# ofrikleinfeld/ObjectPermanence

Measured on AMD Instinct MI355X. Metric: CATER clips/sec (300f x 10obj) OPNet inference, higher is better.
Workload: dtype f32

## Files before the change

include/opnet_hip.h:

```cpp
#ifndef OPNET_HIP_H
#define OPNET_HIP_H

#include <stddef.h>
#include <stdint.h>

#ifdef __cplusplus
extern "C" {
#endif

#define OPNET_OK 0
#define OPNET_EINVAL (-1)
#define OPNET_ESHAPE (-2)
#define OPNET_EWORKSPACE (-3)
#define OPNET_EHIP (-4)

#define OPNET_SLOTS 15
#define OPNET_FEATS 6

#define OPNET_HIP_ABI_VERSION 9
int opnet_hip_abi_version(void);
const char *opnet_last_error(void);

size_t opnet_packed_weights_bytes(int H1, int H2);
int opnet_pack_weights_f32(const float *w_ih1, const float *w_hh1, const float *w_sel,
                           const float *w_ih2, const float *w_hh2, const float *w_out,
                           float *packed, size_t packed_bytes, int H1, int H2, void *stream);

size_t opnet_workspace_bytes(int B, int T, int H1, int H2);
int opnet_forward_f32(const float *boxes, const float *packed, float *y, float *logits,
                      void *workspace, size_t workspace_bytes, int B, int T, int H1, int H2,
                      void *stream);

typedef struct opnet_plan opnet_plan;
int opnet_plan_create(opnet_plan **plan, int B, int T, int H1, int H2);
int opnet_plan_forward(opnet_plan *plan, const float *boxes, const float *packed, float *y,
                       float *logits, void *workspace, size_t workspace_bytes, void *stream);
void opnet_plan_destroy(opnet_plan *plan);

int opnet_xcd_max_batch(void);
int opnet_xcd_supported(int H1, int H2);
size_t opnet_xcd_workspace_bytes(int B, int T, int H1, int H2);
int opnet_xcd_forward_f32(const float *boxes, const float *packed, float *y, float *logits,
                          void *workspace, size_t workspace_bytes, int B, int T, int H1, int H2,
                          void *stream);
int opnet_xcd_forward_multi_f32(const float *const *boxes, const int *counts, int nreq, const float *packed, float *y,
                                float *logits, void *workspace, size_t workspace_bytes, int T, int H1, int H2, void *stream);
int opnet_xcd_profile(int enable);
int opnet_xcd_profile_read(double *kernel_ms_total, int *launches);
int opnet_kernel_profile_read(int tag, double *kernel_ms_total, int *launches);
void opnet_xcd_set_trace(void *device_buffer);
int opnet_xcd4_max_batch(void);
size_t opnet_xcd4_packed_weights_bytes(int H1, int H2);
size_t opnet_xcd4_workspace_bytes(int B, int T, int H1, int H2);
int opnet_xcd4_pack_weights_f32(const float *w_ih1, const float *w_hh1, const float *w_sel, const float *w_ih2,
                                const float *w_hh2, const float *w_out, float *packed, size_t packed_bytes,
                                int H1, int H2, void *stream);
int opnet_xcd4_forward_f32(const float *boxes, const float *packed, float *y, float *logits, void *workspace,
                           size_t workspace_bytes, int B, int T, int H1, int H2, void *stream);
void opnet_xcd4_set_trace(void *device_buffer);
int opnet_xcd4_last_status(unsigned *out4);
size_t opnet_xcd4_status_offset(int B, int T, int H1, int H2);
size_t opnet_train_status_offset(int B, int T, int H1, int H2);
void opnet_xcd4_enable(int on);
int opnet_xcd4_enabled(void);

size_t opnet_train_packed_weights_bytes(int H1, int H2);
int opnet_train_pack_weights_f32(const float *w_ih1, const float *w_hh1, const float *w_sel,
                                 const float *w_ih2, const float *w_hh2, const float *w_out,
                                 float *packed, size_t packed_bytes, int H1, int H2, void *stream);
size_t opnet_train_workspace_bytes(int B, int T, int H1, int H2);
int opnet_train_forward_f32(const float *boxes, const float *packed, float *y, float *logits,
                            void *workspace, size_t workspace_bytes, int B, int T, int H1, int H2,
// ... 259 lines not shown
```

objectpermanence_amd/_lib.py:

```python
from __future__ import annotations

import ctypes
import os
from ctypes import POINTER, c_char_p, c_double, c_float, c_int, c_size_t, c_void_p

from . import build as _build

_LIB = None

OPNET_OK = 0
ABI_VERSION = 9
NO_OFFSET = ctypes.c_size_t(-1).value


class OpnetHipError(RuntimeError):
    pass


def _declare(lib):
    fp = c_void_p
    lib.opnet_hip_abi_version.restype = c_int
    lib.opnet_hip_abi_version.argtypes = []
    lib.opnet_last_error.restype = c_char_p
    lib.opnet_last_error.argtypes = []
    lib.opnet_packed_weights_bytes.restype = c_size_t
    lib.opnet_packed_weights_bytes.argtypes = [c_int, c_int]
    lib.opnet_pack_weights_f32.restype = c_int
    lib.opnet_pack_weights_f32.argtypes = [fp, fp, fp, fp, fp, fp, fp, c_size_t, c_int, c_int, c_void_p]
    lib.opnet_workspace_bytes.restype = c_size_t
    lib.opnet_workspace_bytes.argtypes = [c_int, c_int, c_int, c_int]
    lib.opnet_forward_f32.restype = c_int
    lib.opnet_forward_f32.argtypes = [fp, fp, fp, fp, c_void_p, c_size_t, c_int, c_int, c_int, c_int, c_void_p]
    lib.opnet_xcd_max_batch.restype = c_int
    lib.opnet_xcd_max_batch.argtypes = []
    lib.opnet_xcd_supported.restype = c_int
    lib.opnet_xcd_supported.argtypes = [c_int, c_int]
    lib.opnet_xcd_workspace_bytes.restype = c_size_t
    lib.opnet_xcd_workspace_bytes.argtypes = [c_int, c_int, c_int, c_int]
    lib.opnet_xcd_forward_f32.restype = c_int
    lib.opnet_xcd_forward_f32.argtypes = [fp, fp, fp, fp, c_void_p, c_size_t, c_int, c_int, c_int, c_int, c_void_p]
    lib.opnet_xcd_forward_multi_f32.restype = c_int
    lib.opnet_xcd_forward_multi_f32.argtypes = [POINTER(c_void_p), POINTER(c_int), c_int, fp, fp, fp, c_void_p, c_size_t,
                                                c_int, c_int, c_int, c_void_p]
    lib.opnet_xcd_profile.restype = c_int
    lib.opnet_xcd_profile.argtypes = [c_int]
    lib.opnet_xcd_profile_read.restype = c_int
    lib.opnet_xcd_profile_read.argtypes = [POINTER(c_double), POINTER(c_int)]
    lib.opnet_kernel_profile_read.restype = c_int
    lib.opnet_kernel_profile_read.argtypes = [c_int, POINTER(c_double), POINTER(c_int)]
    lib.opnet_xcd_set_trace.restype = None
    lib.opnet_xcd_set_trace.argtypes = [c_void_p]
    lib.opnet_xcd4_max_batch.restype = c_int
    lib.opnet_xcd4_max_batch.argtypes = []
    lib.opnet_xcd4_packed_weights_bytes.restype = c_size_t
    lib.opnet_xcd4_packed_weights_bytes.argtypes = [c_int, c_int]
    lib.opnet_xcd4_workspace_bytes.restype = c_size_t
    lib.opnet_xcd4_workspace_bytes.argtypes = [c_int, c_int, c_int, c_int]
    lib.opnet_xcd4_pack_weights_f32.restype = c_int
    lib.opnet_xcd4_pack_weights_f32.argtypes = [fp, fp, fp, fp, fp, fp, fp, c_size_t, c_int, c_int, c_void_p]
    lib.opnet_xcd4_forward_f32.restype = c_int
    lib.opnet_xcd4_forward_f32.argtypes = [fp, fp, fp, fp, c_void_p, c_size_t, c_int, c_int, c_int, c_int, c_void_p]
    lib.opnet_xcd4_set_trace.restype = None
    lib.opnet_xcd4_set_trace.argtypes = [c_void_p]
    lib.opnet_xcd4_last_status.restype = c_int
    lib.opnet_xcd4_last_status.argtypes = [POINTER(ctypes.c_uint)]
    lib.opnet_plan_create.restype = c_int
    lib.opnet_plan_create.argtypes = [POINTER(c_void_p), c_int, c_int, c_int, c_int]
# ... 254 lines not shown
    lib.opdet_detections_workspace_bytes.restype = c_size_t
    lib.opdet_detections_workspace_bytes.argtypes = [c_int, c_int]
    lib.opdet_detections_f32.restype = c_int
    lib.opdet_detections_f32.argtypes = [fp, fp, fp, fp, c_int, c_int, c_int, c_int, c_int, c_int, c_float, c_float, c_int,
                                         fp, fp, fp, fp, c_void_p, c_size_t, c_void_p]
    lib.opdet_rpn_workspace_bytes_batch.restype = c_size_t
    lib.opdet_rpn_workspace_bytes_batch.argtypes = [c_int, c_int, ip, ip, ip, c_int, c_int, c_int]
    lib.opdet_rpn_proposals_batch_f32.restype = c_int
    lib.opdet_rpn_proposals_batch_f32.argtypes = [POINTER(c_void_p), c_int, c_int, ip, ip, ip, c_int, c_int, c_int, c_int, c_int, c_int,
                                                  c_float, c_float, fp, fp, fp, c_void_p, c_size_t, c_void_p]
    lib.opdet_roi_align_batch_f32.restype = c_int
    lib.opdet_roi_align_batch_f32.argtypes = [POINTER(c_void_p), c_int, ip, ip, c_int, c_int, fp, fp, c_int, fp, c_void_p]
    lib.opdet_detections_workspace_bytes_batch.restype = c_size_t
    lib.opdet_detections_workspace_bytes_batch.argtypes = [c_int, c_int, c_int]
    lib.opdet_detections_batch_f32.restype = c_int
    lib.opdet_detections_batch_f32.argtypes = [fp, fp, fp, fp] + [c_int] * 9 + [c_float, c_float, c_int,
                                               fp, fp, fp, fp, c_void_p, c_size_t, c_void_p]
    lib.opnet_encode_clips_f32.restype = c_int
    lib.opnet_encode_clips_f32.argtypes = [c_void_p, c_void_p, c_void_p, c_void_p, c_void_p, c_int, c_int, c_int, c_void_p, c_int,
                                           c_void_p, c_void_p]
    lib.opnet_load_clips_f32.restype = c_int
    lib.opnet_load_clips_f32.argtypes = [c_void_p, c_void_p, c_int, c_int, c_int, c_void_p, c_int, c_void_p, c_void_p, c_void_p,
                                         c_char_p, c_int]
    lib.opnet_postprocess_iou.restype = c_int
    lib.opnet_postprocess_iou.argtypes = [fp, fp, fp, fp, fp, c_int, c_int, c_void_p]
    lib.opnet_dp_guard_f32.restype = c_int
    lib.opnet_dp_guard_f32.argtypes = [fp, fp, fp, c_float, c_void_p]


EXPORTS = [
    "opnet_hip_abi_version", "opnet_last_error", "opnet_packed_weights_bytes", "opnet_pack_weights_f32",
    "opnet_workspace_bytes", "opnet_forward_f32", "opnet_plan_create", "opnet_plan_forward",
    "opnet_plan_destroy", "opnet_postprocess_iou", "opnet_encode_clips_f32", "opnet_load_clips_f32",
    "opnet_xcd_max_batch", "opnet_xcd_supported", "opnet_xcd_workspace_bytes", "opnet_xcd_forward_f32", "opnet_xcd_forward_multi_f32", "opnet_xcd_set_trace", "opnet_xcd4_set_trace", "opnet_xcd4_last_status", "opnet_xcd4_max_batch", "opnet_xcd4_packed_weights_bytes",
    "opnet_xcd4_workspace_bytes", "opnet_xcd4_pack_weights_f32", "opnet_xcd4_forward_f32",
    "opnet_xcd_profile", "opnet_xcd_profile_read", "opnet_kernel_profile_read",
    "opnet_train_packed_weights_bytes", "opnet_train_pack_weights_f32", "opnet_train_workspace_bytes",
    "opnet_train_forward_f32", "opnet_train_backward_f32", "opnet_train_extra_workspace_bytes", "opnet_train_backward_ex_f32",
    "opnet_selection_ce_f32", "opnet_l1_loss_f32", "opnet_smooth_l1_loss_f32", "opnet_adam_step_f32", "opnet_adam_multi_step_f32",
    "opnet_adam_multi_step_guarded_f32", "opnet_dp_guard_f32", "opnet_xcd4_status_offset", "opnet_train_status_offset", "opnet_xcd4_enable", "opnet_xcd4_enabled",
    "opnet_mlp_pack_weights_f32", "opnet_mlp_forward_f32",
    "opnet_stream_state_floats", "opnet_stream_workspace_bytes", "opnet_stream_step_f32", "opnet_stream_step_ragged_f32",
    "opnet_stream_x4_max_streams", "opnet_stream_x4_workspace_bytes", "opnet_stream_x4_status_offset",
    "opnet_stream_step_x4_f32",
    "opnet_online_encode_f32", "opnet_online_encode_ragged_f32",
    "opnet_mlp_train_pack_weights_f32", "opnet_mlp_train_forward_f32", "opnet_mlp_train_backward_f32",
    "opnet_mlp_train_backward_ex_f32", "opnet_train_forward_state_f32", "opnet_train_backward_state_f32",
    "opseq_lstm_stack_packed_bytes", "opseq_lstm_stack_workspace_bytes", "opseq_lstm_stack_pack_weights_f32",
    "opseq_lstm_stack_forward_f32", "opseq_lstm_stack_forward_graph_f32", "opseq_graph_cache_clear",
    "opseq_stream_state_floats", "opseq_stream_workspace_bytes", "opseq_stream_step_f32", "opseq_stream_step_ragged_f32",
    "opseq_stream_input_product_f32",
    "opseq_stream_x_max_streams", "opseq_stream_x_workspace_bytes", "opseq_stream_x_status_offset", "opseq_stream_step_x_f32",
    "opseq_xcd_supported", "opseq_xcd_enable", "opseq_xcd_max_batch", "opseq_xcd_packed_bytes", "opseq_xcd_workspace_bytes",
    "opseq_xcd_status_offset", "opseq_xcd_pack_weights_f32", "opseq_xcd_forward_f32", "opseq_lstm_stack_train_status_offset", "opseq_xcd_set_trace",
    "opseq_xcdt_supported", "opseq_xcdt_enable", "opseq_xcdt_max_batch", "opseq_xcdt_packed_bytes", "opseq_xcdt_workspace_bytes",
    "opseq_xcdt_status_offset", "opseq_xcdt_pack_weights_f32", "opseq_xcdt_forward_f32", "opseq_xcdt_set_trace",
    "opseq_slot_embed_relu_f32", "opseq_slot_embed_relu_bwd_f32", "opseq_slot_embed_bwd_workspace_bytes", "opseq_slot_embed_relu_bwd_ws_f32",
    "opseq_lstm_stack_train_packed_bytes", "opseq_lstm_stack_train_workspace_bytes",
    "opseq_lstm_stack_train_pack_weights_f32", "opseq_lstm_stack_train_forward_f32",
    "opseq_lstm_stack_train_backward_f32",
    "opseq_encoder_workspace_bytes",
    "opseq_encoder_layer_f32", "opseq_encoder_layer_segmented_f32", "opseq_encoder_layer_batched_f32", "opseq_ffn_fused_supported", "opseq_ffn_fused_plan", "opseq_ffn_fused_f32", "opseq_attention_f32", "opseq_attention_workspace_bytes",
    "opseq_encoder_train_saved_bytes", "opseq_encoder_train_scratch_bytes", "opseq_encoder_layer_train_forward_f32",
    "opseq_encoder_layer_train_backward_f32", "opseq_encoder_test_masks_set", "opseq_encoder_test_masks_clear",
    "opdet_conv2d_f32", "opdet_conv2d_workspace_bytes", "opdet_conv2d_ws_f32", "opdet_wino_weights_bytes", "opdet_wino_weights_f32", "opdet_conv2d_wino_workspace_bytes", "opdet_conv2d_wino_f32", "opdet_conv2d_up_f32", "opdet_conv2d_dual_workspace_bytes", "opdet_conv2d_dual_f32", "opdet_maxpool3x3s2_f32", "opdet_subsample2_f32", "opdet_upsample_add_f32",
    "opdet_preprocess_frame_f32", "opdet_rpn_workspace_bytes", "opdet_rpn_proposals_f32", "opdet_roi_align_f32",
    "opdet_detections_workspace_bytes", "opdet_detections_f32", "opdet_rpn_workspace_bytes_batch", "opdet_rpn_proposals_batch_f32",
# ... 33 lines not shown
```

objectpermanence_amd/csrc/opnet_abi.hip:

```cpp
#include "opnet_kernels.hip"
#include "opnet_xcd_kernels.hip"
#include "opnet_xcd_split_kernels.hip"
#include "opnet_train_kernels.hip"
#include "opnet_state_train_kernels.hip"
#include "opnet_xcd4_kernels.hip"
#include "seq_kernels.hip"
#include "seq_xcd_kernels.hip"
#include "seq_xcdt_kernels.hip"
#include "seq_xcd_bwd_kernels.hip"
#include "conv_kernels.hip"
#include "wino_kernels.hip"
#include "ffn_kernels.hip"
#include "attn_kernels.hip"
#include "enc_train_kernels.hip"
#include "attn_train_kernels.hip"
#include "opnet_stream_kernels.hip"
#include "opnet_stream_x4_kernels.hip"
#include "seq_stream_kernels.hip"
#include "seq_stream_x_kernels.hip"
#include "online_encode_kernels.hip"

#include <stdarg.h>
#include <stdlib.h>
#include <stdio.h>
// ... 292 lines not shown
static int xcd_ring_mode() { return env_int("OPNET_XCD_RING", 1) != 0; }
static int xcd_head_once(int NGT) { return env_int("OPNET_XCD_HO", (NGT + XCD_COUNT - 1) / XCD_COUNT >= 3 ? 1 : 0) != 0; }
static int xcd_split_mode() { return env_int("OPNET_XCD_SPLIT", 1) != 0; }
static int xcd_pgather_mode() { return env_int("OPNET_XCD_PGATHER", 1) != 0; }
static int xcd_head_once_split() { return env_int("OPNET_XCD_HO", 1) != 0; }

static XcdWorkspaceLayout xcd_workspace_layout(int B, int T, bool infer = false)
{
    XcdWorkspaceLayout L;
    const size_t NGT = (size_t)(B + 15) / 16;
    size_t o = 0;
    L.NGT = (int)NGT;
    L.ring = xcd_ring_mode();
    L.ho = infer && xcd_split_mode() ? xcd_head_once_split() : xcd_head_once(L.NGT);
    const size_t NS = L.ring ? (size_t)XCD_RING : (size_t)(T + 1);
    L.status = o; o += 2048;
    L.flags = o;  o += align_up(NGT * XCD_CUS * 4, 256);
    L.xp = o;     o += NGT * (size_t)(T + 2) * OPNET_KXQ * 256;
    L.h1h = o;    o += NGT * NS * (XCD_H1 / 4) * 256;
    L.h2h = o;    o += NGT * NS * (XCD_H2 / 4) * 256;
    L.fbh = o;    o += NGT * NS * 1024;
    L.yp = o;     if (L.ring && !L.ho) o += NGT * (size_t)T * XCD_CUS * 256;
    L.wsp = L.xs = L.fbs = 0;
    if (infer && L.ho) {
        o = align_up(o, 256);
        L.wsp = o; o += align_up(packed_layout(XCD_H1, XCD_H2).total * 4, 256);
        L.xs = o;  o += NGT * (size_t)(T + 2) * OPNET_KXQ * 256;
        L.fbs = o; o += NGT * NS * 2048;
    }
    L.total = align_up(o, 256);
    return L;
}

#define XCD_MAX_B (XCD_COUNT * XCD_NGMAX * 16)

static int check_xcd(int B, int T, int H1, int H2)
{
    if (B <= 0 || T <= 0) return fail(OPNET_ESHAPE, "B=%d T=%d must be positive", B, T);
    if (H1 != XCD_H1 || H2 != XCD_H2)
        return fail(OPNET_ESHAPE, "the per-XCD persistent forward is built for H1=%d, H2=%d (got %d, %d); use opnet_forward_f32",
                    XCD_H1, XCD_H2, H1, H2);
    if (B > XCD_MAX_B) return fail(OPNET_ESHAPE, "B=%d > %d clips per launch: split the batch", B, XCD_MAX_B);
    const XcdWorkspaceLayout L = xcd_workspace_layout(B, T, true);
    if (L.total >= ((size_t)1 << 31))
        return fail(OPNET_ESHAPE, "B=%d x T=%d: the workspace exceeds the 2 GiB one buffer descriptor addresses; split the batch", B, T);
    return OPNET_OK;
}

extern "C" int opnet_xcd_max_batch(void) { return XCD_MAX_B; }

extern "C" size_t opnet_xcd_workspace_bytes(int B, int T, int H1, int H2)
{
    if (check_xcd(B, T, H1, H2)) return 0;
    return xcd_workspace_layout(B, T, true).total;
}

static unsigned long long *g_xcd_trace = nullptr;
extern "C" void opnet_xcd_set_trace(void *device_buffer) { g_xcd_trace = (unsigned long long *)device_buffer; }

static std::mutex g_xcd_mu;
static hipEvent_t g_xcd_done[64] = {};
#define BWD_MAX_SLICES 4
struct BwdSide {
    hipStream_t s[BWD_MAX_SLICES - 1];
    hipEvent_t fork, join[BWD_MAX_SLICES - 1];
};
static BwdSide g_bwd_side[64] = {};
static int g_xcd_cus[64] = {};

#define PROF_XCD 0
#define PROF_SEQX 1
#define PROF_ATTN 2
#define PROF_SEQT 3
#define PROF_FFN 4
#define PROF_ATTN_TF 5
// ... 62 lines not shown
    std::lock_guard<std::mutex> lock(g_xcd_mu);
    if (!g_xcd_cus[dev]) {
        hipDeviceProp_t prop;
        if (hipGetDeviceProperties(&prop, dev) != hipSuccess) return 0;
        g_xcd_cus[dev] = prop.multiProcessorCount;
    }
    return g_xcd_cus[dev];
}

static bool whole_device(int dev) { return xcd_device_cus(dev) >= XCD_COUNT * XCD_CUS; }
static bool whole_device()
{
    int dev = 0;
    return hipGetDevice(&dev) == hipSuccess && whole_device(dev);
}

static int persistent_device(int *dev)
{
    HIP_TRY(hipGetDevice(dev));
    if (!whole_device(*dev))
        return fail(OPNET_ESHAPE, "device %d exposes %d CUs; a persistent launch needs %d resident workgroups", *dev,
                    xcd_device_cus(*dev), XCD_COUNT * XCD_CUS);
    return OPNET_OK;
}

template <class Launch>
static int persistent_launch(int dev, hipStream_t st, int tag, Launch launch)
{
    if (dev < 0 || dev >= 64) return fail(OPNET_EINVAL, "device index %d out of range", dev);
    std::lock_guard<std::mutex> lock(g_xcd_mu);
    if (!g_xcd_done[dev]) HIP_TRY(hipEventCreateWithFlags(&g_xcd_done[dev], hipEventDisableTiming));
    else HIP_TRY(hipStreamWaitEvent(st, g_xcd_done[dev], 0));
    ProfPair pe{};
    const bool prof = tag >= 0 && prof_begin(st, &pe);
    launch();
    if (prof) prof_end(tag, st, pe);
    HIP_TRY(hipEventRecord(g_xcd_done[dev], st));
    return OPNET_OK;
}

extern "C" int opnet_xcd_supported(int H1, int H2)
{
    if (H1 != XCD_H1 || H2 != XCD_H2) return 0;
    return whole_device() ? 1 : 0;
}

static XcdArgs make_xcd_args(const XcdWorkspaceLayout &L, size_t base, size_t status, int B, int T, const float *packed, char *w,
                             float *y, float *logits)
{
    XcdArgs a;
    memset(&a, 0, sizeof(a));
    a.B = B; a.T = T; a.NGT = L.NGT;
    a.packed = packed;
    a.xp = (const float4 *)(w + base + L.xp);
    a.h1h = (float4 *)(w + base + L.h1h);
    a.h2h = (float4 *)(w + base + L.h2h);
    a.fbh = (float4 *)(w + base + L.fbh);
    a.flags = (unsigned *)(w + base + L.flags);
    a.status = (unsigned *)(w + status);
    a.logits = logits;
    a.ws = w;
    a.xp_off = (unsigned)(base + L.xp); a.h1_off = (unsigned)(base + L.h1h); a.h2_off = (unsigned)(base + L.h2h);
    a.fb_off = (unsigned)(base + L.fbh); a.flags_off = (unsigned)(base + L.flags); a.status_off = (unsigned)status;
    a.ring = L.ring; a.yp_off = (unsigned)(base + L.yp); a.y = y;
    a.force_safe = env_int("OPNET_XCD_SAFE", 0);
    a.debug = env_int("OPNET_XCD_DEBUG", 0);
    return a;
}

template <bool TRAIN>
static int xcd_forward_launch(const XcdSources &src, const XcdArgs &a, bool ho, int dev, hipStream_t st)
{
    opnet_xcd_pack_input<<<dim3(a.T + 2, a.NGT), 384, 0, st>>>(src, a);
    if (int rc = persistent_launch(dev, st, PROF_XCD, [&] {
            if (ho) opnet_xcd_forward<true, TRAIN><<<XCD_COUNT * XCD_CUS, 512, 0, st>>>(a);
            else opnet_xcd_forward<false, TRAIN><<<XCD_COUNT * XCD_CUS, 512, 0, st>>>(a);
        }))
        return rc;
    if (a.ring && ho)
        opnet_xcd_y_poison<<<64, 256, 0, st>>>(a, a.y);
    else if (a.ring)
        opnet_xcd_y_reduce<<<ew_blocks((long)a.NGT * a.T * 16, 2048), 256, 0, st>>>(a, a.y);
    else
        opnet_xcd_out_head<<<dim3(a.T, a.NGT), 256, 0, st>>>(a, a.y);
    HIP_TRY(hipGetLastError());
    return OPNET_OK;
}

static int xcd_forward_launch_split(const XcdSources &src, const XcdArgs &a0, const XcdWorkspaceLayout &L, int dev, hipStream_t st)
{
    XcdSplitArgs s;
    memset(&s, 0, sizeof(s));
    s.a = a0;
    s.a.fbh = (float4 *)(a0.ws + L.fbs);
    s.a.fb_off = (unsigned)L.fbs;
    s.wsp = a0.ws + L.wsp;
    s.xs_off = (unsigned)L.xs;
    s.pgather = xcd_pgather_mode();
    const PackedLayout P = packed_layout(XCD_H1, XCD_H2);
    const long lanes = (long)((P.wih2p + (P.total - P.wselp)) / 512) * 64;
    s.wsp_blocks = (unsigned)((lanes + 255) / 256);
    opnet_xcd_split_weights<<<s.wsp_blocks, 256, 0, st>>>(s);
    opnet_xcd_pack_input_split<<<dim3(s.a.T + 2, s.a.NGT), 384, 0, st>>>(src, s);
    if (int rc = persistent_launch(dev, st, PROF_XCD, [&] { opnet_xcd_forward_split<<<XCD_COUNT * XCD_CUS, 512, 0, st>>>(s); }))
        return rc;
    if (s.a.ring) opnet_xcd_y_poison<<<64, 256, 0, st>>>(s.a, s.a.y);
    else opnet_xcd_out_head_split<<<dim3(s.a.T, s.a.NGT), 256, 0, st>>>(s.a, s.a.y);
    HIP_TRY(hipGetLastError());
    return OPNET_OK;
}

static int xcd_forward_impl(const XcdSources &src, const float *packed, float *y, float *logits,
                            void *workspace, size_t workspace_bytes, int B, int T, int H1, int H2,
                            void *stream)
{
    if (int rc = check_xcd(B, T, H1, H2)) return rc;
    if (!packed || !y || !logits || !workspace) return fail(OPNET_EINVAL, "null pointer");
    if (!aligned16(packed) || !aligned16(y) || !aligned16(workspace))
        return fail(OPNET_EINVAL, "packed/y/workspace must be 16-byte aligned");
    const XcdWorkspaceLayout L = xcd_workspace_layout(B, T, true);
    if (workspace_bytes < L.total) return fail(OPNET_EWORKSPACE, "workspace %zu B < %zu B", workspace_bytes, L.total);
    int dev = 0;
    if (int rc = persistent_device(&dev)) return rc;
    XcdArgs a = make_xcd_args(L, 0, L.status, B, T, packed, (char *)workspace, y, logits);
    a.trace = g_xcd_trace;
    if (L.ho && xcd_split_mode()) return xcd_forward_launch_split(src, a, L, dev, (hipStream_t)stream);
    return xcd_forward_launch<false>(src, a, L.ho, dev, (hipStream_t)stream);
}

extern "C" int opnet_xcd_forward_f32(const float *boxes, const float *packed, float *y, float *logits,
                                     void *workspace, size_t workspace_bytes, int B, int T, int H1, int H2,
                                     void *stream)
{
    if (!boxes) return fail(OPNET_EINVAL, "null pointer");
    if (((uintptr_t)boxes) & 7u) return fail(OPNET_EINVAL, "boxes must be 8-byte aligned");
    XcdSources src;
    memset(&src, 0, sizeof(src));
// ... 175 lines not shown
}

struct TrainPackedLayout {
    size_t fwd_total, w2bt, w1bt, wih2t, wsel, wout, x4fwd, x4bwd, total;
};

static bool x4_dims(int H1, int H2) { return H1 == XCD_H1 && H2 == XCD_H2; }

static TrainPackedLayout train_packed_layout(int H1, int H2)
{
    TrainPackedLayout L;
    size_t o = packed_layout(H1, H2).total;
    L.fwd_total = o;
    o = align_up(o, 4);
    L.w2bt = o;  o += (size_t)(H2 / 16) * (H2 / 4) * 256;
    L.w1bt = o;  o += (size_t)(H1 / 16) * (H1 / 4) * 256;
    L.wih2t = o; o += (size_t)(H2 / 4) * 256;
    L.wsel = o;  o += align_up((size_t)OPNET_SLOTS * H1, 4);
    L.wout = o;  o += align_up((size_t)4 * H2, 4);
    L.x4fwd = o; o += x4_dims(H1, H2) ? x4_packed_layout().total : 0;
    L.x4bwd = o; o += x4_dims(H1, H2) ? x4b_packed_layout().total : 0;
    L.total = o;
    return L;
}

struct TrainWorkspaceLayout {
    size_t io, xp, state, h1all, c1all, h2all, c2all, state_end, x2all, g1, g2, psave, ystage, lgstage,
        dyp, dlall, dhpart2, dhpart1, dx2part, dcz, dc2, dc1, dcz_end, l1part, x4h1x, x4h2x, x4status, x4da1x, x4da2x, x4dfx, wgpart,
        xcdws, total;
};
#define WG2_MAX_WAVES 1024

static bool x4_batch(int B, int H1, int H2) { return x4_dims(H1, H2) && (B + 31) / 32 <= X4_NGMAX; }
static bool xcdt_batch(int B, int H1, int H2) { return x4_dims(H1, H2) && B > 96 && B <= XCD_MAX_B; }

static TrainWorkspaceLayout train_workspace_layout(int B, int T, int H1, int H2)
{
    const size_t RB = (B + 31) / 32, TT = T;
    TrainWorkspaceLayout L;
    size_t o = 0;
    L.io = o;      o += align_up(sizeof(OpnetIO), 256);
    L.xp = o;      o += TT * RB * OPNET_KXQ * 32 * 16;
    L.state = o;
    L.h1all = o;   o += (TT + 1) * RB * (size_t)H1 * 32 * 4;
    L.c1all = o;   o += (TT + 1) * RB * (size_t)H1 * 32 * 4;
    L.h2all = o;   o += (TT + 1) * RB * (size_t)H2 * 32 * 4;
    L.c2all = o;   o += (TT + 1) * RB * (size_t)H2 * 32 * 4;
    L.state_end = o;
    L.x2all = o;   o += TT * RB * 64 * 16;
    L.g1 = o;      o += TT * RB * (size_t)H1 * 32 * 16;
    L.g2 = o;      o += TT * RB * (size_t)H2 * 32 * 16;
    L.psave = o;   o += TT * RB * 128 * 16;
    L.ystage = o;  o += RB * 32 * TT * 16;
    L.lgstage = o; o += RB * 32 * TT * OPNET_SLOTS * 4;
    L.dyp = o;     o += TT * RB * 32 * 16;
    L.dlall = o;   o += TT * RB * 128 * 16;
    L.dhpart2 = o; o += 4 * RB * (size_t)H2 * 32 * 4;
    L.dhpart1 = o; o += 4 * RB * (size_t)H1 * 32 * 4;
    L.dx2part = o; o += 4 * RB * 16 * 32 * 4;
    L.dcz = o;
    L.dc2 = o;     o += RB * (size_t)H2 * 32 * 4;
    L.dc1 = o;     o += RB * (size_t)H1 * 32 * 4;
    L.dcz_end = o;
    L.l1part = o;  o += 1024 * 4;
    o = align_up(o, 4096);
    const size_t NG = x4_batch(B, H1, H2) ? RB * 8 : 0;
    L.x4h1x = o;   o += NG * X4_SLOTS * 4096;
// ... 2388 lines not shown
```

objectpermanence_amd/csrc/opnet_xcd_kernels.hip:

```cpp
#include <hip/hip_runtime.h>
#include <stdint.h>

#include <type_traits>

#include "opnet_ctx.h"

#define XCD_COUNT 8
#define XCD_CUS 32
#define XCD_NGMAX 8
#define XCD_H1 256
#define XCD_H2 512
#define XCD_RING 4
#define XCD_SPIN_LIMIT 150000000ll

#define XB_X0 0
#define XB_H1 (6 * 64)
#define XB_H2 (22 * 64)
#define XB_FB (54 * 64)
#define XB_F4 (55 * 64)
#define XB_CHUNKS 55

struct XcdArgs {
    int B, T, NGT;
    const float *packed;
// ... 30 lines not shown
    unsigned keep;
    asm volatile("s_mov_b32 %0, m0\n\ts_mov_b32 m0, %4\n\ts_nop 2\n\tbuffer_load_dwordx4 %1, %2, %3 offen sc1 lds\n\ts_mov_b32 m0, %0"
                 : "=&s"(keep) : "v"(voff), "s"(rsrc), "s"(soff), "s"(lds_dst) : "memory");
}

__device__ __forceinline__ void xcd_store16(__amdgpu_buffer_rsrc_t r, unsigned voff, unsigned soff, float4 v, bool local)
{
    xcd_u32x4 u;
    u.x = __float_as_uint(v.x); u.y = __float_as_uint(v.y); u.z = __float_as_uint(v.z); u.w = __float_as_uint(v.w);
    if (local) __builtin_amdgcn_raw_buffer_store_b128(u, r, voff, soff, 0);
    else __builtin_amdgcn_raw_buffer_store_b128(u, r, voff, soff, 16);
}
__device__ __forceinline__ void xcd_st4(__amdgpu_buffer_rsrc_t r, unsigned voff, unsigned soff, float4 v)
{
    xcd_u32x4 u;
    u.x = __float_as_uint(v.x); u.y = __float_as_uint(v.y); u.z = __float_as_uint(v.z); u.w = __float_as_uint(v.w);
    __builtin_amdgcn_raw_buffer_store_b128(u, r, voff, soff, 0);
}
__device__ __forceinline__ void xcd_st1(__amdgpu_buffer_rsrc_t r, unsigned voff, unsigned soff, float v)
{
    __builtin_amdgcn_raw_buffer_store_b32(__float_as_uint(v), r, voff, soff, 0);
}
__device__ __forceinline__ void xcd_store4(__amdgpu_buffer_rsrc_t r, unsigned voff, unsigned soff, float v, bool local)
{
    if (local) __builtin_amdgcn_raw_buffer_store_b32(__float_as_uint(v), r, voff, soff, 0);
    else __builtin_amdgcn_raw_buffer_store_b32(__float_as_uint(v), r, voff, soff, 16);
}
__device__ __forceinline__ void xcd_store_flag(unsigned *p, unsigned v, bool local)
{
    if (local) __hip_atomic_store(p, v, __ATOMIC_RELAXED, __HIP_MEMORY_SCOPE_WAVEFRONT);
    else __hip_atomic_store(p, v, __ATOMIC_RELAXED, __HIP_MEMORY_SCOPE_AGENT);
}

#define XCD_MAX_SOURCES 64
struct XcdSources {
    const float *p[XCD_MAX_SOURCES];
    int start[XCD_MAX_SOURCES + 1];
    int n;
};

__global__ void __launch_bounds__(384) opnet_xcd_pack_input(const XcdSources src, XcdArgs a)
{
    const int slot = blockIdx.x, gg = blockIdx.y;
    const int T = a.T, tid = threadIdx.x;
    const float4 z = make_float4(0.f, 0.f, 0.f, 0.f);
    {
        const int kq = tid % OPNET_KXQ, clip = tid / OPNET_KXQ;
        const int b = gg * 16 + clip, t = slot - 1;
        float4 v = z;
        if (b < a.B && t >= 0 && t < T) {
            int r = 0;
            while (r + 1 < src.n && b >= src.start[r + 1]) ++r;
            const float2 *s2 = (const float2 *)(src.p[r] + ((long)(b - src.start[r]) * T + t) * OPNET_KX + kq * 4);
            const int k = kq * 4;
            if (k + 1 < OPNET_KX) { float2 p = s2[0]; v.x = p.x; v.y = p.y; }
            if (k + 3 < OPNET_KX) { float2 q = s2[1]; v.z = q.x; v.w = q.y; }
        }
        ((float4 *)a.xp)[(((long)gg * (T + 2) + slot) * OPNET_KXQ + kq) * 16 + clip] = v;
    }
    if (slot == 0) {
        const long NS = a.ring ? XCD_RING : T + 1;
        float4 *h1 = a.h1h + (long)gg * NS * (XCD_H1 * 4);
        float4 *h2 = a.h2h + (long)gg * NS * (XCD_H2 * 4);
        for (int i = tid; i < XCD_H1 * 4; i += 384) h1[i] = z;
        for (int i = tid; i < XCD_H2 * 4; i += 384) h2[i] = z;
        if (tid < 64) a.fbh[(long)gg * NS * 64 + tid] = z;
        if (tid < XCD_CUS) a.flags[gg * XCD_CUS + tid] = 0u;
        if (gg == 0 && tid < 8) a.status[tid] = 0u;
        if (gg == 0 && tid < XCD_COUNT * XCD_CUS) a.status[8 + tid] = 0xffffffffu;
    }
}

__device__ __forceinline__ bool xcd_flags_ready(const unsigned *flags, unsigned need)
{
    const unsigned v = __hip_atomic_load(flags + (threadIdx.x & 31), __ATOMIC_RELAXED, __HIP_MEMORY_SCOPE_AGENT);
    return __all(v >= need);
}

__device__ __forceinline__ bool xcd_wait_flags(const unsigned *flags, unsigned need, unsigned *status, int phase)
{
    if (xcd_flags_ready(flags, need)) return true;
    const int lane = threadIdx.x & 63;
    long long t0 = 0;
    for (unsigned spins = 1;; ++spins) {
        __builtin_amdgcn_s_sleep(4);
// ... 643 lines not shown
    }
}


__global__ void __launch_bounds__(256) opnet_xcd_y_reduce(const XcdArgs a, float *__restrict__ y)
{
    const long total = (long)a.NGT * a.T * 16;
    const float4 *yp = (const float4 *)(a.ws + a.yp_off);
    const bool bad = a.status[0] != 0u;
    for (long i = blockIdx.x * 256L + threadIdx.x; i < total; i += (long)gridDim.x * 256) {
        const int n = (int)(i & 15);
        const long gt = i >> 4;
        const float4 *p = yp + gt * (XCD_CUS * 16) + n;
        float4 sum = p[0];
        for (int cu = 1; cu < XCD_CUS; ++cu) {
            const float4 v = p[cu * 16];
            sum.x += v.x; sum.y += v.y; sum.z += v.z; sum.w += v.w;
        }
        if (bad) sum = make_float4(NAN, NAN, NAN, NAN);
        const long gg = gt / a.T, t = gt - gg * a.T;
        const long b = gg * 16 + n;
        if (b < a.B) ((float4 *)y)[b * a.T + t] = sum;
    }
}


__global__ void __launch_bounds__(256) opnet_xcd_y_poison(const XcdArgs a, float *__restrict__ y)
{
    if (a.status[0] == 0u) return;
    const long total = (long)a.B * a.T;
    for (long i = blockIdx.x * 256L + threadIdx.x; i < total; i += (long)gridDim.x * 256)
        ((float4 *)y)[i] = make_float4(NAN, NAN, NAN, NAN);
}
```

objectpermanence_amd/csrc/opnet_xcd_split_kernels.hip:

```cpp
#define XS_SCALE 2048.f
#define XS_ISCALE (1.f / 2048.f)
#define XS_RANGE 32768.f
#define XS_ABORT_RANGE 3u
#define XS_CHUNKS 56
#define XS_F8 (XS_CHUNKS * 64)
#define XS_H1 (6 * 64)
#define XS_H2 (22 * 64)

typedef _Float16 xs_h8 __attribute__((ext_vector_type(8)));
typedef _Float16 xs_h4 __attribute__((ext_vector_type(4)));
typedef unsigned xs_u32x2 __attribute__((ext_vector_type(2)));

struct XcdSplitArgs {
    XcdArgs a;
    const char *wsp;
    unsigned xs_off;
    unsigned wsp_blocks;
    int pgather;
};

__device__ __forceinline__ void xs_split(float v, _Float16 *hi, _Float16 *lo)
{
    const _Float16 h = (_Float16)v;
    *hi = h;
// ... 15 lines not shown
        const float4 v0 = src[0], v1 = src[16];
        const float v[8] = {v0.x, v0.y, v0.z, v0.w, v1.x, v1.y, v1.z, v1.w};
        xs_h8 hi, lo;
#pragma unroll
        for (int j = 0; j < 8; ++j) {
            _Float16 h, q;
            xs_split(v[j], &h, &q);
            hi[j] = h; lo[j] = q;
            bad |= !xs_in_range(v[j]);
        }
        xs_h8 *dst = (xs_h8 *)(s.wsp + base * 4) + l;
        dst[0] = hi;
        dst[64] = lo;
    }
    if (i < (long)(P.wselp - P.wih2p)) bad |= !xs_in_range(s.a.packed[P.wih2p + i]);
    const int any = __syncthreads_or(bad ? 1 : 0);
    if (threadIdx.x == 0) ((unsigned *)(s.wsp + P.wih2p * 4))[blockIdx.x] = any ? 1u : 0u;
    if (blockIdx.x == 0) {
        if (threadIdx.x < 8) s.a.status[threadIdx.x] = 0u;
        s.a.status[8 + threadIdx.x] = 0xffffffffu;
    }
}

__global__ void __launch_bounds__(384) opnet_xcd_pack_input_split(const XcdSources src, const XcdSplitArgs s)
{
    const XcdArgs &a = s.a;
    const int slot = blockIdx.x, gg = blockIdx.y;
    const int T = a.T, tid = threadIdx.x;
    const float4 z = make_float4(0.f, 0.f, 0.f, 0.f);
    bool bad = false;
    {
        const int kq = tid % OPNET_KXQ, clip = tid / OPNET_KXQ;
        const int b = gg * 16 + clip, t = slot - 1;
        float4 v = z;
        if (b < a.B && t >= 0 && t < T) {
            int r = 0;
            while (r + 1 < src.n && b >= src.start[r + 1]) ++r;
            const float2 *s2 = (const float2 *)(src.p[r] + ((long)(b - src.start[r]) * T + t) * OPNET_KX + kq * 4);
            const int k = kq * 4;
            if (k + 1 < OPNET_KX) { float2 p = s2[0]; v.x = p.x; v.y = p.y; }
            if (k + 3 < OPNET_KX) { float2 q = s2[1]; v.z = q.x; v.w = q.y; }
        }
        const long sl = (long)gg * (T + 2) + slot;
        ((float4 *)a.xp)[(sl * OPNET_KXQ + kq) * 16 + clip] = v;
        xs_h4 hi, lo;
        const float vv[4] = {v.x, v.y, v.z, v.w};
#pragma unroll
        for (int j = 0; j < 4; ++j) {
            _Float16 h, q;
            xs_split(vv[j], &h, &q);
            hi[j] = h; lo[j] = q;
            bad |= !xs_in_range(vv[j]);
        }
        char *d = a.ws + s.xs_off + sl * (OPNET_KXQ * 256) + (kq >> 3) * 2048 + ((((kq >> 1) & 3) * 16 + clip) * 16) + (kq & 1) * 8;
        *(xs_h4 *)d = hi;
        *(xs_h4 *)(d + 1024) = lo;
    }
    const long NS = a.ring ? XCD_RING : T + 1;
    for (long fs = slot; fs < NS; fs += T + 2)
        if (tid < 128) ((float4 *)(a.ws + a.fb_off))[((long)gg * NS + fs) * 128 + tid] = z;
    if (slot == 0) {
        float4 *h1 = a.h1h + (long)gg * NS * (XCD_H1 * 4);
        float4 *h2 = a.h2h + (long)gg * NS * (XCD_H2 * 4);
        for (int i = tid; i < XCD_H1 * 4; i += 384) h1[i] = z;
        for (int i = tid; i < XCD_H2 * 4; i += 384) h2[i] = z;
        if (tid < XCD_CUS) a.flags[gg * XCD_CUS + tid] = 0u;
        if (gg == 0) {
            const PackedLayout P = packed_layout(XCD_H1, XCD_H2);
            const unsigned *wb = (const unsigned *)(s.wsp + P.wih2p * 4);
            for (unsigned i = tid; i < s.wsp_blocks; i += 384) bad |= wb[i] != 0u;
// ... 477 lines not shown
```

objectpermanence_amd/learned_models.py:

```python
from __future__ import annotations

import math
import os
from typing import Dict, Tuple

import torch
import torch.nn as nn

from . import _lib
from ._device_cache import PackedImages, TrainingBuffers, Workspaces, check_weights
from .launch_monitor import LaunchMonitor


class AbstractCaterModel(nn.Module):

    def __init__(self, config: Dict[str, int]):
        super().__init__()
        self.config: Dict[str, int] = config
        self.max_objects_in_frame = 15
        self.bb_in_dim = 5
        self.bb_out_dim = 4

    def launch_guard(self):
        r = getattr(self, "_runner", None)
# ... 444 lines not shown
    def _forward_xcd4(self, boxes: torch.Tensor, stream: int):
        lib = _lib.load()
        B, T, dev = int(boxes.shape[0]), int(boxes.shape[1]), boxes.device
        x4packed = self._x4_packed_weights(dev, stream)
        ws = self._x4ws.get(stream, (B, T), dev, (lib.opnet_xcd4_workspace_bytes, B, T, self._h1, self._h2))
        y = torch.empty((B, T, 4), dtype=torch.float32, device=dev)
        logits = torch.empty((B, 15, T), dtype=torch.float32, device=dev)
        _lib.check(lib.opnet_xcd4_forward_f32(boxes.data_ptr(), x4packed.data_ptr(), y.data_ptr(), logits.data_ptr(),
                                              ws.data_ptr(), ws.numel(), B, T, self._h1, self._h2, stream),
                   "opnet_xcd4_forward_f32")
        self._monitor.watch(ws, lib.opnet_xcd4_status_offset(B, T, self._h1, self._h2),
                            lambda: self._redo_on_chain(boxes, y, logits), "opnet_xcd4_forward")
        return y, logits

    def _forward_xcd(self, boxes: torch.Tensor, packed: torch.Tensor, stream: int):
        lib = _lib.load()
        B, T, dev = int(boxes.shape[0]), int(boxes.shape[1]), boxes.device
        y = torch.empty((B, T, 4), dtype=torch.float32, device=dev)
        logits = torch.empty((B, 15, T), dtype=torch.float32, device=dev)
        step = int(lib.opnet_xcd_max_batch())
        while step > 64 and lib.opnet_xcd_workspace_bytes(min(step, B), T, self._h1, self._h2) == 0:
            step //= 2
        for lo in range(0, B, step):
            n = min(step, B - lo)
            ws = self._xws.get(stream, (n, T), dev, (lib.opnet_xcd_workspace_bytes, n, T, self._h1, self._h2))
            rc = lib.opnet_xcd_forward_f32(boxes[lo:lo + n].data_ptr(), packed.data_ptr(), y[lo:lo + n].data_ptr(),
                                           logits[lo:lo + n].data_ptr(), ws.data_ptr(), ws.numel(), n, T,
                                           self._h1, self._h2, stream)
            _lib.check(rc, "opnet_xcd_forward_f32")
            self._monitor.watch(ws, 0, lambda b=boxes[lo:lo + n], yy=y[lo:lo + n], ll=logits[lo:lo + n]:
                                self._redo_on_chain(b, yy, ll), "opnet_xcd_forward")
        return y, logits

    def forward_requests(self, requests):
        lib = _lib.load()
        B = sum(int(r.shape[0]) for r in requests)
        ok = (len(requests) > 1 and len(requests) <= 64 and not torch.is_grad_enabled() and all(r.is_cuda for r in requests)
              and not self._wants_xcd4(B) and self._wants_xcd(B) and B <= int(lib.opnet_xcd_max_batch())
              and all(r.dim() == 4 and r.shape[1:] == requests[0].shape[1:] and r.device == requests[0].device for r in requests))
        if not ok:
            return self(requests[0] if len(requests) == 1 else torch.cat(list(requests), dim=0))
        reqs = [r if (r.is_contiguous() and r.dtype == torch.float32) else r.contiguous().float() for r in requests]
        T, dev = int(reqs[0].shape[1]), reqs[0].device
        if reqs[0].shape[2] != 15 or reqs[0].shape[3] != 6:
            raise ValueError(f"boxes must be [B, T, 15, 6], got {tuple(reqs[0].shape)}")
        with torch.cuda.device(dev):
            packed = self._packed_weights(dev)
            stream = _stream_ptr(dev)
            if lib.opnet_xcd_workspace_bytes(B, T, self._h1, self._h2) == 0:
                return self(torch.cat(reqs, dim=0))
            ws = self._xws.get(stream, (B, T), dev, (lib.opnet_xcd_workspace_bytes, B, T, self._h1, self._h2))
            y = torch.empty((B, T, 4), dtype=torch.float32, device=dev)
            logits = torch.empty((B, 15, T), dtype=torch.float32, device=dev)
            n = len(reqs)
            ptrs = (_lib.c_void_p * n)(*[r.data_ptr() for r in reqs])
            counts = (_lib.ctypes.c_int * n)(*[int(r.shape[0]) for r in reqs])
            _lib.check(lib.opnet_xcd_forward_multi_f32(ptrs, counts, n, packed.data_ptr(), y.data_ptr(), logits.data_ptr(),
                                                       ws.data_ptr(), ws.numel(), T, self._h1, self._h2, stream),
                       "opnet_xcd_forward_multi_f32")
            self._monitor.watch(ws, 0, lambda: self._redo_on_chain(torch.cat(reqs, dim=0), y, logits), "opnet_xcd_forward")
        return y, logits

    def xcd_status(self):
        return {k: ws[:12].view(torch.int32).tolist() for k, ws in self._xws.items()}

    def zero_state(self, B: int):
        return _zero_state(self, B)

    def forward(self, boxes: torch.Tensor, logits_grad: bool = False, state=None, return_state: bool = False):
        if not boxes.is_cuda:
# ... 616 lines not shown
```

Measured before the change: 254,800.

## Run oversized XCD batches as multiple persistent-kernel rounds inside one call

```diff
diff --git a/include/opnet_hip.h b/include/opnet_hip.h
--- a/include/opnet_hip.h
+++ b/include/opnet_hip.h
@@ -38,6 +38,7 @@
 void opnet_plan_destroy(opnet_plan *plan);
 
 int opnet_xcd_max_batch(void);
+int opnet_xcd_round_plan(int B, int *first_group, int *groups, int capacity);
 int opnet_xcd_supported(int H1, int H2);
 size_t opnet_xcd_workspace_bytes(int B, int T, int H1, int H2);
 int opnet_xcd_forward_f32(const float *boxes, const float *packed, float *y, float *logits,
diff --git a/objectpermanence_amd/_lib.py b/objectpermanence_amd/_lib.py
--- a/objectpermanence_amd/_lib.py
+++ b/objectpermanence_amd/_lib.py
@@ -33,6 +33,8 @@
     lib.opnet_forward_f32.argtypes = [fp, fp, fp, fp, c_void_p, c_size_t, c_int, c_int, c_int, c_int, c_void_p]
     lib.opnet_xcd_max_batch.restype = c_int
     lib.opnet_xcd_max_batch.argtypes = []
+    lib.opnet_xcd_round_plan.restype = c_int
+    lib.opnet_xcd_round_plan.argtypes = [c_int, POINTER(c_int), POINTER(c_int), c_int]
     lib.opnet_xcd_supported.restype = c_int
     lib.opnet_xcd_supported.argtypes = [c_int, c_int]
     lib.opnet_xcd_workspace_bytes.restype = c_size_t
@@ -353,7 +355,7 @@
     "opnet_hip_abi_version", "opnet_last_error", "opnet_packed_weights_bytes", "opnet_pack_weights_f32",
     "opnet_workspace_bytes", "opnet_forward_f32", "opnet_plan_create", "opnet_plan_forward",
     "opnet_plan_destroy", "opnet_postprocess_iou", "opnet_encode_clips_f32", "opnet_load_clips_f32",
-    "opnet_xcd_max_batch", "opnet_xcd_supported", "opnet_xcd_workspace_bytes", "opnet_xcd_forward_f32", "opnet_xcd_forward_multi_f32", "opnet_xcd_set_trace", "opnet_xcd4_set_trace", "opnet_xcd4_last_status", "opnet_xcd4_max_batch", "opnet_xcd4_packed_weights_bytes",
+    "opnet_xcd_max_batch", "opnet_xcd_round_plan", "opnet_xcd_supported", "opnet_xcd_workspace_bytes", "opnet_xcd_forward_f32", "opnet_xcd_forward_multi_f32", "opnet_xcd_set_trace", "opnet_xcd4_set_trace", "opnet_xcd4_last_status", "opnet_xcd4_max_batch", "opnet_xcd4_packed_weights_bytes",
     "opnet_xcd4_workspace_bytes", "opnet_xcd4_pack_weights_f32", "opnet_xcd4_forward_f32",
     "opnet_xcd_profile", "opnet_xcd_profile_read", "opnet_kernel_profile_read",
     "opnet_train_packed_weights_bytes", "opnet_train_pack_weights_f32", "opnet_train_workspace_bytes",
diff --git a/objectpermanence_amd/csrc/opnet_abi.hip b/objectpermanence_amd/csrc/opnet_abi.hip
--- a/objectpermanence_amd/csrc/opnet_abi.hip
+++ b/objectpermanence_amd/csrc/opnet_abi.hip
@@ -348,7 +348,31 @@
     return L;
 }
 
-#define XCD_MAX_B (XCD_COUNT * XCD_NGMAX * 16)
+#define XCD_LAUNCH_GROUPS (XCD_COUNT * XCD_NGMAX)
+#define XCD_LAUNCH_B (XCD_LAUNCH_GROUPS * 16)
+#define XCD_MAX_ROUNDS 4
+#define XCD_MAX_B (XCD_MAX_ROUNDS * XCD_LAUNCH_B)
+
+static int xcd_round_plan(int NGT, int *first, int *groups)
+{
+    const int R = (NGT + XCD_LAUNCH_GROUPS - 1) / XCD_LAUNCH_GROUPS;
+    const int base = R ? NGT / R : 0, rem = R ? NGT % R : 0;
+    for (int r = 0, g = 0; r < R; ++r) {
+        first[r] = g;
+        groups[r] = base + (r < rem ? 1 : 0);
+        g += groups[r];
+    }
+    return R;
+}
+
+extern "C" int opnet_xcd_round_plan(int B, int *first_group, int *groups, int capacity)
+{
+    if (B <= 0 || B > XCD_MAX_B || !first_group || !groups) return 0;
+    int f[XCD_MAX_ROUNDS], n[XCD_MAX_ROUNDS];
+    const int R = xcd_round_plan((B + 15) / 16, f, n);
+    for (int r = 0; r < R && r < capacity; ++r) { first_group[r] = f[r]; groups[r] = n[r]; }
+    return R;
+}
 
 static int check_xcd(int B, int T, int H1, int H2)
 {
@@ -356,7 +380,7 @@
     if (H1 != XCD_H1 || H2 != XCD_H2)
         return fail(OPNET_ESHAPE, "the per-XCD persistent forward is built for H1=%d, H2=%d (got %d, %d); use opnet_forward_f32",
                     XCD_H1, XCD_H2, H1, H2);
-    if (B > XCD_MAX_B) return fail(OPNET_ESHAPE, "B=%d > %d clips per launch: split the batch", B, XCD_MAX_B);
+    if (B > XCD_MAX_B) return fail(OPNET_ESHAPE, "B=%d > %d clips per call: split the batch", B, XCD_MAX_B);
     const XcdWorkspaceLayout L = xcd_workspace_layout(B, T, true);
     if (L.total >= ((size_t)1 << 31))
         return fail(OPNET_ESHAPE, "B=%d x T=%d: the workspace exceeds the 2 GiB one buffer descriptor addresses; split the batch", B, T);
@@ -485,9 +509,11 @@
     if (!g_xcd_done[dev]) HIP_TRY(hipEventCreateWithFlags(&g_xcd_done[dev], hipEventDisableTiming));
     else HIP_TRY(hipStreamWaitEvent(st, g_xcd_done[dev], 0));
     ProfPair pe{};
-    const bool prof = tag >= 0 && prof_begin(st, &pe);
-    launch();
-    if (prof) prof_end(tag, st, pe);
+    bool prof = tag >= 0 && prof_begin(st, &pe);
+    auto prof_close = [&] { if (prof) { prof_end(tag, st, pe); prof = false; } };
+    if constexpr (std::is_invocable_v<Launch, decltype(prof_close) &>) launch(prof_close);
+    else launch();
+    prof_close();
     HIP_TRY(hipEventRecord(g_xcd_done[dev], st));
     return OPNET_OK;
 }
@@ -521,13 +547,49 @@
     return a;
 }
 
+static XcdArgs xcd_round_view(const XcdArgs &a, int g0, int n, size_t fb_slot)
+{
+    XcdArgs v = a;
+    const size_t G = (size_t)g0, T = (size_t)a.T, NS = a.ring ? (size_t)XCD_RING : T + 1;
+    const size_t xp = G * (T + 2) * OPNET_KXQ * 256, h1 = G * NS * (XCD_H1 / 4) * 256, h2 = G * NS * (XCD_H2 / 4) * 256;
+    const size_t fb = G * NS * fb_slot, fl = G * XCD_CUS * 4, yp = G * T * XCD_CUS * 256;
+    v.NGT = n;
+    v.B = a.B - g0 * 16 < n * 16 ? a.B - g0 * 16 : n * 16;
+    v.xp = (const float4 *)((const char *)a.xp + xp);  v.xp_off = a.xp_off + (unsigned)xp;
+    v.h1h = (float4 *)((char *)a.h1h + h1);            v.h1_off = a.h1_off + (unsigned)h1;
+    v.h2h = (float4 *)((char *)a.h2h + h2);            v.h2_off = a.h2_off + (unsigned)h2;
+    v.fbh = (float4 *)((char *)a.fbh + fb);            v.fb_off = a.fb_off + (unsigned)fb;
+    v.flags = (unsigned *)((char *)a.flags + fl);      v.flags_off = a.flags_off + (unsigned)fl;
+    v.yp_off = a.yp_off + (unsigned)yp;
+    v.y = a.y + G * 16 * T * 4;
+    v.logits = a.logits + G * 16 * OPNET_SLOTS * T;
+    if (g0) v.trace = nullptr;
+    return v;
+}
+
+template <class LaunchRound>
+static int xcd_run_rounds(const XcdArgs &a, int dev, hipStream_t st, LaunchRound launch_round)
+{
+    int first[XCD_MAX_ROUNDS], groups[XCD_MAX_ROUNDS];
+    if (a.NGT > XCD_MAX_ROUNDS * XCD_LAUNCH_GROUPS) return fail(OPNET_ESHAPE, "%d groups exceed %d rounds", a.NGT, XCD_MAX_ROUNDS);
+    const int R = xcd_round_plan(a.NGT, first, groups);
+    return persistent_launch(dev, st, PROF_XCD, [&](auto &prof_close) {
+        for (int r = 0; r < R; ++r) {
+            if (r) opnet_xcd_reset_placement<<<1, XCD_COUNT * XCD_CUS, 0, st>>>(a.status);
+            launch_round(first[r], groups[r]);
+            if (r == 0 && a.trace) prof_close();
+        }
+    });
+}
+
 template <bool TRAIN>
 static int xcd_forward_launch(const XcdSources &src, const XcdArgs &a, bool ho, int dev, hipStream_t st)
 {
     opnet_xcd_pack_input<<<dim3(a.T + 2, a.NGT), 384, 0, st>>>(src, a);
-    if (int rc = persistent_launch(dev, st, PROF_XCD, [&] {
-            if (ho) opnet_xcd_forward<true, TRAIN><<<XCD_COUNT * XCD_CUS, 512, 0, st>>>(a);
-            else opnet_xcd_forward<false, TRAIN><<<XCD_COUNT * XCD_CUS, 512, 0, st>>>(a);
+    if (int rc = xcd_run_rounds(a, dev, st, [&](int g0, int n) {
+            const XcdArgs v = xcd_round_view(a, g0, n, 1024);
+            if (ho) opnet_xcd_forward<true, TRAIN><<<XCD_COUNT * XCD_CUS, 512, 0, st>>>(v);
+            else opnet_xcd_forward<false, TRAIN><<<XCD_COUNT * XCD_CUS, 512, 0, st>>>(v);
         }))
         return rc;
     if (a.ring && ho)
@@ -555,7 +617,12 @@
     s.wsp_blocks = (unsigned)((lanes + 255) / 256);
     opnet_xcd_split_weights<<<s.wsp_blocks, 256, 0, st>>>(s);
     opnet_xcd_pack_input_split<<<dim3(s.a.T + 2, s.a.NGT), 384, 0, st>>>(src, s);
-    if (int rc = persistent_launch(dev, st, PROF_XCD, [&] { opnet_xcd_forward_split<<<XCD_COUNT * XCD_CUS, 512, 0, st>>>(s); }))
+    if (int rc = xcd_run_rounds(s.a, dev, st, [&](int g0, int n) {
+            XcdSplitArgs v = s;
+            v.a = xcd_round_view(s.a, g0, n, 2048);
+            v.xs_off = s.xs_off + (unsigned)((size_t)g0 * (size_t)(s.a.T + 2) * OPNET_KXQ * 256);
+            opnet_xcd_forward_split<<<XCD_COUNT * XCD_CUS, 512, 0, st>>>(v);
+        }))
         return rc;
     if (s.a.ring) opnet_xcd_y_poison<<<64, 256, 0, st>>>(s.a, s.a.y);
     else opnet_xcd_out_head_split<<<dim3(s.a.T, s.a.NGT), 256, 0, st>>>(s.a, s.a.y);
@@ -797,7 +864,7 @@
 #define WG2_MAX_WAVES 1024
 
 static bool x4_batch(int B, int H1, int H2) { return x4_dims(H1, H2) && (B + 31) / 32 <= X4_NGMAX; }
-static bool xcdt_batch(int B, int H1, int H2) { return x4_dims(H1, H2) && B > 96 && B <= XCD_MAX_B; }
+static bool xcdt_batch(int B, int H1, int H2) { return x4_dims(H1, H2) && B > 96 && B <= XCD_LAUNCH_B; }
 
 static TrainWorkspaceLayout train_workspace_layout(int B, int T, int H1, int H2)
 {
diff --git a/objectpermanence_amd/csrc/opnet_xcd_kernels.hip b/objectpermanence_amd/csrc/opnet_xcd_kernels.hip
--- a/objectpermanence_amd/csrc/opnet_xcd_kernels.hip
+++ b/objectpermanence_amd/csrc/opnet_xcd_kernels.hip
@@ -86,12 +86,28 @@
     else __hip_atomic_store(p, v, __ATOMIC_RELAXED, __HIP_MEMORY_SCOPE_AGENT);
 }
 
-#define XCD_MAX_SOURCES 64
+#define XCD_MAX_SOURCES 256
 struct XcdSources {
     const float *p[XCD_MAX_SOURCES];
     int start[XCD_MAX_SOURCES + 1];
     int n;
 };
+
+__device__ __forceinline__ int xcd_source_of_group(const XcdSources &src, int b0)
+{
+    int lo = 0, hi = src.n - 1;
+    while (lo < hi) {
+        const int mid = (lo + hi + 1) >> 1;
+        if (src.start[mid] <= b0) lo = mid;
+        else hi = mid - 1;
+    }
+    return __builtin_amdgcn_readfirstlane(lo);
+}
+__device__ __forceinline__ int xcd_source_of_clip(const XcdSources &src, int r, int b)
+{
+    while (r + 1 < src.n && b >= src.start[r + 1]) ++r;
+    return r;
+}
 
 __global__ void __launch_bounds__(384) opnet_xcd_pack_input(const XcdSources src, XcdArgs a)
 {
@@ -101,10 +117,10 @@
     {
         const int kq = tid % OPNET_KXQ, clip = tid / OPNET_KXQ;
         const int b = gg * 16 + clip, t = slot - 1;
+        const int r0 = t >= 0 && t < T ? xcd_source_of_group(src, gg * 16) : 0;
         float4 v = z;
         if (b < a.B && t >= 0 && t < T) {
-            int r = 0;
-            while (r + 1 < src.n && b >= src.start[r + 1]) ++r;
+            const int r = xcd_source_of_clip(src, r0, b);
             const float2 *s2 = (const float2 *)(src.p[r] + ((long)(b - src.start[r]) * T + t) * OPNET_KX + kq * 4);
             const int k = kq * 4;
             if (k + 1 < OPNET_KX) { float2 p = s2[0]; v.x = p.x; v.y = p.y; }
@@ -814,3 +830,8 @@
     for (long i = blockIdx.x * 256L + threadIdx.x; i < total; i += (long)gridDim.x * 256)
         ((float4 *)y)[i] = make_float4(NAN, NAN, NAN, NAN);
 }
+
+__global__ void __launch_bounds__(256) opnet_xcd_reset_placement(unsigned *__restrict__ status)
+{
+    status[8 + threadIdx.x] = 0xffffffffu;
+}
diff --git a/objectpermanence_amd/csrc/opnet_xcd_split_kernels.hip b/objectpermanence_amd/csrc/opnet_xcd_split_kernels.hip
--- a/objectpermanence_amd/csrc/opnet_xcd_split_kernels.hip
+++ b/objectpermanence_amd/csrc/opnet_xcd_split_kernels.hip
@@ -71,10 +71,10 @@
     {
         const int kq = tid % OPNET_KXQ, clip = tid / OPNET_KXQ;
         const int b = gg * 16 + clip, t = slot - 1;
+        const int r0 = t >= 0 && t < T ? xcd_source_of_group(src, gg * 16) : 0;
         float4 v = z;
         if (b < a.B && t >= 0 && t < T) {
-            int r = 0;
-            while (r + 1 < src.n && b >= src.start[r + 1]) ++r;
+            const int r = xcd_source_of_clip(src, r0, b);
             const float2 *s2 = (const float2 *)(src.p[r] + ((long)(b - src.start[r]) * T + t) * OPNET_KX + kq * 4);
             const int k = kq * 4;
             if (k + 1 < OPNET_KX) { float2 p = s2[0]; v.x = p.x; v.y = p.y; }
diff --git a/objectpermanence_amd/learned_models.py b/objectpermanence_amd/learned_models.py
--- a/objectpermanence_amd/learned_models.py
+++ b/objectpermanence_amd/learned_models.py
@@ -500,10 +500,12 @@
                                 self._redo_on_chain(b, yy, ll), "opnet_xcd_forward")
         return y, logits
 
+    XCD_MAX_REQUESTS = 256
+
     def forward_requests(self, requests):
         lib = _lib.load()
         B = sum(int(r.shape[0]) for r in requests)
-        ok = (len(requests) > 1 and len(requests) <= 64 and not torch.is_grad_enabled() and all(r.is_cuda for r in requests)
+        ok = (len(requests) > 1 and len(requests) <= self.XCD_MAX_REQUESTS and not torch.is_grad_enabled() and all(r.is_cuda for r in requests)
               and not self._wants_xcd4(B) and self._wants_xcd(B) and B <= int(lib.opnet_xcd_max_batch())
               and all(r.dim() == 4 and r.shape[1:] == requests[0].shape[1:] and r.device == requests[0].device for r in requests))
         if not ok:
```

Result: slower. 250,700 (-1.6%).
